# EugenHotaj/zig_gpt2

Hardware: AMD Instinct MI355X
Metric: tokens/sec GPT-2-124M greedy 1024-ctx (higher is better)
Workload: dtype bf16 weights, f32 activations/accumulate; 1 GPU; GPT-2 124M greedy decode, 1 prompt(s)/GPU x 1 GPU(s), 1-token prompts, 1024 decode steps per prompt (reference generate loop, src/main.zig:322-342); vocab=50257, context=1024, n_layer=12, n_heads=12, n_embed=768, prompts_per_gpu=1, global_prompts=1, kv_cache=f32, hip_graph=True, l2_prefetcher=on, parallelism=replicated weights, prompts sharded x1, RCCL broadcast at start-up only

## Files before the change

### zig_gpt2_amd/csrc/elementwise.hip

```cpp
#include <algorithm>

#include "zg_kernels.h"

namespace zg {

namespace {

__device__ __forceinline__ float block_allsum(float v, float* s_red) {
    v = wave_allsum(v);
    const int lane = threadIdx.x & 63, wave = threadIdx.x >> 6, nw = blockDim.x >> 6;
    __syncthreads();
    if (lane == 0) s_red[wave] = v;
    __syncthreads();
    float t = 0.0f;
    for (int w = 0; w < nw; ++w) t += s_red[w];
    return t;
}

__device__ __forceinline__ float block_allmax(float v, float* s_red) {
    v = wave_allmax(v);
    const int lane = threadIdx.x & 63, wave = threadIdx.x >> 6, nw = blockDim.x >> 6;
    __syncthreads();
    if (lane == 0) s_red[wave] = v;
    __syncthreads();
// ... 147 lines not shown
        out[r * n_embed + e] = in[r * 3 * n_embed + split_idx * n_embed + e];
}

__global__ __launch_bounds__(64) void transpose_kernel(const float* in, size_t t, size_t n, size_t h, float* out) {
    const size_t s = blockIdx.x, hh = blockIdx.y, b = blockIdx.z;
    const float* src = in + b * t * n * h + s * n * h + hh * h;
    float* dst = out + b * t * n * h + hh * t * h + s * h;
    for (size_t d = threadIdx.x; d < h; d += blockDim.x) dst[d] = src[d];
}

__global__ __launch_bounds__(256) void copy_kernel(const float* in, float* out, size_t n) {
    const size_t stride = (size_t)gridDim.x * blockDim.x;
    for (size_t i = (size_t)blockIdx.x * blockDim.x + threadIdx.x; i < n; i += stride) out[i] = in[i];
}

__global__ __launch_bounds__(256) void f32_to_bf16_kernel(const float* in, bf16_t* out, size_t n) {
    const size_t stride = (size_t)gridDim.x * blockDim.x;
    for (size_t i = (size_t)blockIdx.x * blockDim.x + threadIdx.x; i < n; i += stride)
        out[i] = f32_to_bf16_rne(in[i]);
}

__global__ __launch_bounds__(256) void split3_kernel(const float* __restrict__ in, bf16_t* __restrict__ out, size_t rows, int K) {
    const size_t quads = rows * (size_t)(K / 4), stride = (size_t)gridDim.x * blockDim.x;
    for (size_t i = (size_t)blockIdx.x * blockDim.x + threadIdx.x; i < quads; i += stride) {
        const size_t r = i / (K / 4), k = (i % (K / 4)) * 4;
        const f32x4 v = *reinterpret_cast<const f32x4*>(in + r * K + k);
        uint32_t h0, m0, l0, h1, m1, l1;
        split3_pk(v.x, v.y, h0, m0, l0);
        split3_pk(v.z, v.w, h1, m1, l1);
        bf16_t* o = out + r * (size_t)(3 * K) + k;
        *reinterpret_cast<u32x2*>(o) = u32x2{h0, h1};
        *reinterpret_cast<u32x2*>(o + K) = u32x2{m0, m1};
        *reinterpret_cast<u32x2*>(o + 2 * K) = u32x2{l0, l1};
    }
}

__device__ __forceinline__ f32x4 load_b24x4(const void* w, size_t row, int K, int k) {
    const char* r = reinterpret_cast<const char*>(w) + row * (size_t)(3 * K);
    const u32x2 h = *reinterpret_cast<const u32x2*>(r + 2 * (size_t)k);
    const uint32_t l = *reinterpret_cast<const uint32_t*>(r + 2 * (size_t)K + k);
    return f32x4{__uint_as_float((h.x << 16) | ((l & 0xffu) << 8)), __uint_as_float((h.x & 0xffff0000u) | (l & 0xff00u)),
                 __uint_as_float((h.y << 16) | ((l >> 8) & 0xff00u)), __uint_as_float((h.y & 0xffff0000u) | ((l >> 16) & 0xff00u))};
}

__global__ __launch_bounds__(256) void f32_to_b24_kernel(const float* __restrict__ in, size_t rows, int K, char* __restrict__ out) {
    const size_t per_row = (size_t)(K / 8), n = rows * per_row;
    for (size_t i = blockIdx.x * (size_t)blockDim.x + threadIdx.x; i < n; i += (size_t)gridDim.x * blockDim.x) {
        const size_t r = i / per_row, k = (i % per_row) * 8;
        const f32x4 a = *reinterpret_cast<const f32x4*>(in + r * K + k);
        const f32x4 b = *reinterpret_cast<const f32x4*>(in + r * K + k + 4);
        const float v[8] = {a.x, a.y, a.z, a.w, b.x, b.y, b.z, b.w};
        uint32_t q[8];
#pragma unroll
        for (int j = 0; j < 8; ++j) q[j] = b24_round(v[j]);
        char* o = out + r * (size_t)(3 * K);
        *reinterpret_cast<u32x4*>(o + 2 * k) = u32x4{(q[0] >> 8) | ((q[1] >> 8) << 16), (q[2] >> 8) | ((q[3] >> 8) << 16),
                                                     (q[4] >> 8) | ((q[5] >> 8) << 16), (q[6] >> 8) | ((q[7] >> 8) << 16)};
        *reinterpret_cast<u32x2*>(o + 2 * (size_t)K + k) =
            u32x2{(q[0] & 0xffu) | (q[1] & 0xffu) << 8 | (q[2] & 0xffu) << 16 | (q[3] & 0xffu) << 24,
                  (q[4] & 0xffu) | (q[5] & 0xffu) << 8 | (q[6] & 0xffu) << 16 | (q[7] & 0xffu) << 24};
    }
}

__global__ __launch_bounds__(256) void b24_split3_kernel(const char* __restrict__ in, size_t rows, int K, bf16_t* __restrict__ out) {
    const size_t per_row = (size_t)(K / 4), n = rows * per_row, total = rows * (size_t)K;
    for (size_t i = blockIdx.x * (size_t)blockDim.x + threadIdx.x; i < n; i += (size_t)gridDim.x * blockDim.x) {
        const size_t r = i / per_row, k = (i % per_row) * 4;
        const f32x4 v = load_b24x4(in, r, K, (int)k);
        uint32_t h0, m0, l0, h1, m1, l1;
        split3_pk(v.x, v.y, h0, m0, l0);
        split3_pk(v.z, v.w, h1, m1, l1);
        bf16_t* o = out + r * K + k;
        *reinterpret_cast<u32x2*>(o) = u32x2{h0, h1};
        *reinterpret_cast<u32x2*>(o + total) = u32x2{m0, m1};
        *reinterpret_cast<u32x2*>(o + 2 * total) = u32x2{l0, l1};
    }
}

__device__ __forceinline__ float load_emb(const void* w, int wt, size_t off) {
    if (wt == WT_BF16) return __uint_as_float((uint32_t)reinterpret_cast<const bf16_t*>(w)[off] << 16);
    return reinterpret_cast<const float*>(w)[off];
}

__global__ __launch_bounds__(512) void embed_step_kernel(const EmbedArgs a) {
    __shared__ int s_tok[8];
    const int lane = threadIdx.x & 63, wave = threadIdx.x >> 6;
    const int s = a.ctrl->step;
    const int mode = a.ctrl->mode;
    const int npart = a.n_partials;
    const int n_waves = a.batch > 4 ? 8 : 4;
    for (int b = wave; b < a.batch; b += n_waves) {
        float bv = -3.0e38f;
        int bi = 0x7fffffff;
        for (int base = 0; base < npart; base += 512) {
            float pv[8];
            int pi[8];
#pragma unroll
            for (int j = 0; j < 8; ++j) {
                const int p = min(base + lane + 64 * j, npart - 1);
                pv[j] = a.part_val[(size_t)b * a.part_stride + p];
                pi[j] = a.part_idx[(size_t)b * a.part_stride + p];
            }
#pragma unroll
            for (int j = 0; j < 8; ++j) {
                if (pv[j] > bv || (pv[j] == bv && pi[j] < bi)) { bv = pv[j]; bi = pi[j]; }
            }
        }
        {
            ZG_PIN(a.forced); ZG_PIN(a.wte); ZG_PIN(a.wpe); ZG_PIN(a.weight_type); ZG_PIN(a.n_embed); ZG_PIN(a.cur_token); ZG_PIN(a.out_tokens);
            ZG_PIN(a.out_stride); ZG_PIN(a.x); ZG_PIN(a.pl_out); ZG_PIN(a.pl_g); ZG_PIN(a.epoch); ZG_PIN(a.finish_only); ZG_PIN(a.st_out); ZG_PIN(a.vocab);
        }
        if (b == 0 && a.progress != nullptr && a.finish_only == 0 && lane == 0) {
            const unsigned xcc = __builtin_amdgcn_s_getreg((3 << 11) | 20) & 7u;
            const unsigned long long word = ((unsigned long long)(0x100u | xcc) << 32) | (((unsigned)(s + 1) << 8) | 1u);
            __hip_atomic_store(static_cast<unsigned long long*>(__builtin_assume_aligned(a.progress, 8)), word, __ATOMIC_RELAXED,
                               __HIP_MEMORY_SCOPE_AGENT);
#ifdef ZG_STAMPS
            reinterpret_cast<PfCtl*>(a.progress)->xcd_log[0] = 0x100u | xcc;
#endif
        }
        const int np = a.prompt_len ? a.prompt_len[b] : 0;
        const int p_cur = a.prompt[(size_t)b * a.prompt_stride + min(s, a.prompt_stride - 1)];
        const int p_last = a.prompt[(size_t)b * a.prompt_stride + max(min(np, a.prompt_stride) - 1, 0)];
        const int forced = a.forced[b];
        const int drawn = a.sampled[b];
#define ZG_AM_STEP(N)                                                                                                   \
    {                                                                                                                   \
        const float ov = dpp_row_ror<N>(bv);                                                                            \
        const int oi = __builtin_amdgcn_update_dpp(0, bi, 0x120 | N, 0xF, 0xF, true);                                   \
        if (ov > bv || (ov == bv && oi < bi)) { bv = ov; bi = oi; }                                                     \
    }
        ZG_AM_STEP(8) ZG_AM_STEP(4) ZG_AM_STEP(2) ZG_AM_STEP(1)
#undef ZG_AM_STEP
        {
            const float rv = bv;
            const int ri = bi;
#pragma unroll
            for (int r = 0; r < 64; r += 16) {
                const float ov = lane_value(rv, r);
                const int oi = __builtin_amdgcn_readlane(ri, r);
                if (ov > bv || (ov == bv && oi < bi)) { bv = ov; bi = oi; }
            }
        }
        int g = (unsigned)bi < (unsigned)a.vocab ? bi : 0;
        if (mode == 2 && a.finish_only != 2) g = (unsigned)drawn < (unsigned)a.vocab ? drawn : 0;
        const bool have_pick = a.finish_only == 2 || ((mode != 1) && (s >= 1) && (s - 1 >= np));
        if (lane == 0) {
            if (have_pick) {
                if (a.finish_only == 2) a.cur_token[b] = g;
                else a.out_tokens[(size_t)b * a.out_stride + (s - 1)] = g;
            }
            if (a.finish_only == 0 || a.finish_only == 3) {
                int tok;
                if (mode == 1) tok = forced;
                else if (s < np) tok = p_cur;
                else if (s == np) tok = p_last;
                else tok = g;
                if (mode != 1 && s < np) a.out_tokens[(size_t)b * a.out_stride + s] = tok;
                a.cur_token[b] = tok;
                s_tok[b] = tok;
            }
        }
    }
    if (a.finish_only == 1 || a.finish_only == 2) return;
    __syncthreads();
    const int total4 = a.batch * (a.n_embed >> 2);
    for (int i = threadIdx.x; i < total4; i += 64 * n_waves) {
        const int b = i / (a.n_embed >> 2), e = (i % (a.n_embed >> 2)) * 4;
        const int tok = s_tok[b];
        f32x4 o;
        if (a.weight_type == WT_BF16) {
            const u32x2 t = *reinterpret_cast<const u32x2*>(reinterpret_cast<const bf16_t*>(a.wte) + (size_t)tok * a.n_embed + e);
            const u32x2 p = *reinterpret_cast<const u32x2*>(reinterpret_cast<const bf16_t*>(a.wpe) + (size_t)s * a.n_embed + e);
            o.x = bf16_lo(t.x) + bf16_lo(p.x);
            o.y = bf16_hi(t.x) + bf16_hi(p.x);
            o.z = bf16_lo(t.y) + bf16_lo(p.y);
            o.w = bf16_hi(t.y) + bf16_hi(p.y);
        } else if (a.weight_type == WT_B24) {
            o = load_b24x4(a.wte, (size_t)tok, a.n_embed, e) + load_b24x4(a.wpe, (size_t)s, a.n_embed, e);
        } else {
            const f32x4 t = *reinterpret_cast<const f32x4*>(reinterpret_cast<const float*>(a.wte) + (size_t)tok * a.n_embed + e);
            const f32x4 p = *reinterpret_cast<const f32x4*>(reinterpret_cast<const float*>(a.wpe) + (size_t)s * a.n_embed + e);
            o = t + p;
        }
        *reinterpret_cast<f32x4*>(a.x + (size_t)b * a.n_embed + e) = o;
        if (a.pl_out) {
            const f32x4 v = o * *reinterpret_cast<const f32x4*>(a.pl_g + e);
            uint32_t h0, m0, l0, h1, m1, l1;
            split3_pk(v.x, v.y, h0, m0, l0);
            split3_pk(v.z, v.w, h1, m1, l1);
            *reinterpret_cast<u32x2*>(a.pl_out + plane_elem(0, b, e)) = u32x2{h0, h1};
            *reinterpret_cast<u32x2*>(a.pl_out + plane_elem(1, b, e)) = u32x2{m0, m1};
            *reinterpret_cast<u32x2*>(a.pl_out + plane_elem(2, b, e)) = u32x2{l0, l1};
        }
        if (a.st_out) {
            float s1 = (o.x + o.y) + (o.z + o.w);
            float s2 = fmaf(o.x, o.x, fmaf(o.y, o.y, fmaf(o.z, o.z, o.w * o.w)));
            s1 += __shfl_xor(s1, 1, 64); s2 += __shfl_xor(s2, 1, 64);
            s1 += __shfl_xor(s1, 2, 64); s2 += __shfl_xor(s2, 2, 64);
            if ((threadIdx.x & 3) == 0) *reinterpret_cast<float2*>(a.st_out + ((size_t)b * (a.n_embed >> 4) + (e >> 4)) * 2) = float2{s1, s2};
        }
    }
    if (threadIdx.x == 0 && a.epoch) *a.epoch += 1u;
    if (threadIdx.x == 0 && a.finish_only == 0) {
        a.ctrl->seq_len = s + 1;
        a.ctrl->step = s + 1;
    }
}

constexpr int kSegMax = 4096;

__global__ __launch_bounds__(256) void sample_seg_kernel(const float* __restrict__ logits, int vocab, const SampleParams* params, float inv_temp_arg,
                                                         const float* __restrict__ part_val, int n_part, int part_stride, float* __restrict__ seg_out) {
    __shared__ float s_red[4];
    const int tid = threadIdx.x, lane = tid & 63, wave = tid >> 6, b = blockIdx.y;
    const float inv_temp = params ? params->inv_temp : inv_temp_arg;
    const float* x = logits + (size_t)b * vocab;
    float* so = seg_out + (size_t)b * (kSegMax + 2);
    float mxr = -3.0e38f;
    for (int p = tid; p < n_part; p += 256) mxr = fmaxf(mxr, part_val[(size_t)b * part_stride + p]);
    mxr = wave_allmax(mxr);
    if (lane == 0) s_red[wave] = mxr;
    __syncthreads();
    const float mx = fmaxf(fmaxf(s_red[0], s_red[1]), fmaxf(s_red[2], s_red[3])) * inv_temp;
    const int nseg = (vocab + 63) >> 6;
    for (int sg = blockIdx.x * 4 + wave; sg < nseg; sg += gridDim.x * 4) {
        const int i = sg * 64 + lane;
        const float e = i < vocab ? __expf(x[i] * inv_temp - mx) : 0.0f;
        const float t = wave_allsum(e);
        if (lane == 0) so[sg] = t;
    }
    if (blockIdx.x == 0 && tid == 0) so[kSegMax] = mx;
}

template <bool FILT>
__global__ __launch_bounds__(64) void sample_pick_kernel(const float* __restrict__ logits, int vocab, const SampleParams* params, float inv_temp_arg,
                                                         const float* __restrict__ u_arr, const StepCtrl* ctrl, float* __restrict__ seg_io,
                                                         int* __restrict__ token_out, const float* __restrict__ tau_arr) {
    const int lane = threadIdx.x, b = blockIdx.x;
    const float tau = FILT ? tau_arr[b] : 0.0f;
    const float inv_temp = params ? params->inv_temp : inv_temp_arg;
    const float* x = logits + (size_t)b * vocab;
    float* so = seg_io + (size_t)b * (kSegMax + 2);
    float u;
    if (u_arr) u = u_arr[b];
    else {
        unsigned long long z = params->seed * 0x9E3779B97F4A7C15ULL + (unsigned long long)ctrl->seq_len * 0xD1B54A32D192ED03ULL + (unsigned long long)b + 1ULL;
        z = (z ^ (z >> 30)) * 0xBF58476D1CE4E5B9ULL;
        z = (z ^ (z >> 27)) * 0x94D049BB133111EBULL;
        z ^= z >> 31;
        u = (float)(unsigned)(z >> 40) * 5.9604644775390625e-08f;
    }
    const int nseg = (vocab + 63) >> 6;
    const int run = (nseg + 63) >> 6, s0 = lane * run, s1 = min(s0 + run, nseg);
    const float mx = so[kSegMax];
    float local = 0.0f;
    for (int k = s0; k < s1; ++k) local += so[k];
    float incl = local;
#pragma unroll
    for (int off = 1; off < 64; off <<= 1) {
        const float up = __shfl_up(incl, off, 64);
        if (lane >= off) incl += up;
    }
    const float total = __shfl(incl, 63, 64);
    const float point = u * total;
    int pick = vocab - 1;
    unsigned long long hit = __builtin_amdgcn_ballot_w64(s0 < s1 && point < incl);
    if (hit != 0ull) {
        const int owner = __builtin_ctzll(hit);
        int sg = 0;
        float before = 0.0f;
        if (lane == owner) {
            before = incl - local;
            sg = s1 - 1;
            for (int k = s0; k < s1; ++k) {
                const float v = so[k];
                if (point < before + v) {
                    sg = k;
                    break;
                }
                before += v;
            }
        }
        sg = __shfl(sg, owner, 64);
        before = __shfl(before, owner, 64);
        const int i = sg * 64 + lane;
        const float xi = i < vocab ? x[i] : 0.0f;
        const bool kept = i < vocab && (!FILT || xi >= tau);
        float c = kept ? __expf(FILT ? (xi - mx) * inv_temp : xi * inv_temp - mx) : 0.0f;
// ... 299 lines not shown
                                       2 * kPenMaxHistory * 2 * (int)sizeof(unsigned)));
            raised = true;
        }
    }
    hipLaunchKernelGGL(penalty_apply_kernel, dim3(batch), dim3(256), lds, s, logits, vocab, params, h, slots, counts_out);
    ZG_HIP(hipGetLastError());
    hipLaunchKernelGGL(row_argmax_partials_kernel, dim3(n_part, batch), dim3(256), 0, s, logits, vocab, part_val, part_idx);
    ZG_HIP(hipGetLastError());
    return ZG_OK;
}

static inline int logprob_chunks(int vocab) { return (vocab + kLpChunk - 1) / kLpChunk; }

size_t logprob_workspace_bytes(int batch, int vocab) { return (size_t)batch * logprob_chunks(vocab) * (1 + 2 * kLpTopMax) * 4; }

LogprobWs logprob_workspace(void* base, int batch, int vocab) {
    const size_t slots = (size_t)batch * logprob_chunks(vocab);
    LogprobWs w;
    w.sum = static_cast<float*>(base);
    w.val = w.sum + slots;
    w.idx = reinterpret_cast<int*>(w.val + slots * kLpTopMax);
    return w;
}

int launch_logprob(const float* logits, int batch, int vocab, const float* part_val, const int* part_idx, int n_part, int part_stride, const int* top_n,
                   const LogprobWs& ws, const int* tokens, const StepCtrl* ctrl, const int* prompt_len, const LogprobRec& rec, hipStream_t s) {
    ZG_REQUIRE(vocab >= 1 && vocab <= kLpChunk * kLpMaxChunks, ZG_ERR_UNSUPPORTED, "log-probabilities: vocabulary of %d beyond %d", vocab,
               kLpChunk * kLpMaxChunks);
    ZG_REQUIRE(logits && part_val && (tokens || part_idx) && n_part >= 1 && top_n && ws.sum && rec.logprob && rec.top_ids && rec.top_logprobs &&
                   rec.stride >= 1 && batch >= 1,
               ZG_ERR_ARG, "log-probabilities: missing argument");
    const int nc = logprob_chunks(vocab);
    hipLaunchKernelGGL(logprob_part_kernel, dim3(nc, batch), dim3(256), 0, s, logits, vocab, part_val, n_part, part_stride, top_n, ws, nc);
    ZG_HIP(hipGetLastError());
    hipLaunchKernelGGL(logprob_finish_kernel, dim3(batch), dim3(256), 0, s, logits, vocab, part_val, part_idx, n_part, part_stride, top_n, ws, nc, tokens,
                       ctrl, prompt_len, rec);
    ZG_HIP(hipGetLastError());
    return ZG_OK;
}

size_t score_workspace_bytes(int rows, int vocab) { return (size_t)rows * logprob_chunks(vocab) * (2 + 2 * kLpTopMax) * 4; }

ScoreWs score_workspace(void* base, int rows, int vocab) {
    const size_t slots = (size_t)rows * logprob_chunks(vocab);
    ScoreWs w;
    w.lp.sum = static_cast<float*>(base);
    w.max = w.lp.sum + slots;
    w.lp.val = w.max + slots;
    w.lp.idx = reinterpret_cast<int*>(w.lp.val + slots * kLpTopMax);
    return w;
}

int launch_score(const float* logits, int rows, int vocab, int row_stride, const int* top_n, const ScoreWs& ws, const ScoreTargets& tg, const LogprobRec& rec,
                 hipStream_t s) {
    ZG_REQUIRE(vocab >= 1 && vocab <= kLpChunk * kLpMaxChunks, ZG_ERR_UNSUPPORTED, "score: vocabulary of %d beyond %d", vocab, kLpChunk * kLpMaxChunks);
    ZG_REQUIRE(logits && top_n && ws.lp.sum && tg.tokens && tg.token_stride >= 1 && tg.n >= 1 && tg.past >= 0 && tg.row0 >= 0 && rec.logprob && rec.top_ids &&
                   rec.top_logprobs && rec.stride >= 1 && rows >= 1 && rows <= 65535 && row_stride >= vocab,
               ZG_ERR_ARG, "score: missing argument");
    const int nc = logprob_chunks(vocab);
    hipLaunchKernelGGL(score_part_kernel, dim3(nc, rows), dim3(256), 0, s, logits, vocab, row_stride, top_n, ws, nc);
    ZG_HIP(hipGetLastError());
    hipLaunchKernelGGL(score_finish_kernel, dim3(rows), dim3(256), 0, s, logits, vocab, row_stride, top_n, ws, nc, tg, rec);
    ZG_HIP(hipGetLastError());
    return ZG_OK;
}

int launch_stop(const StopArgs& a, hipStream_t s) {
    ZG_REQUIRE(a.conds && a.tokens && a.prompt_len && a.finish_col && a.reason && a.stride >= 1 && a.batch >= 1 && a.batch <= kStopMaxRows && a.vocab >= 1 &&
                   (a.col >= 0 ? a.col < a.stride : a.ctrl != nullptr) && (a.picks || a.pick_from_record || (a.part_val && a.part_idx && a.n_part >= 1)),
               ZG_ERR_ARG, "stop stage: missing argument");
    hipLaunchKernelGGL(stop_step_kernel, dim3(1), dim3(a.batch > 4 ? 512 : 256), 0, s, a);
    ZG_HIP(hipGetLastError());
    return ZG_OK;
}

int launch_wte_planes(const void* wte, int weight_type, size_t V, size_t V64, int K, bf16_t* out, hipStream_t s) {
    ZG_REQUIRE(wte && out && V >= 1 && V64 >= V && K % 8 == 0 && (weight_type == WT_F32 || weight_type == WT_B24), ZG_ERR_ARG, "wte planes: bad argument");
    hipLaunchKernelGGL(wte_planes_kernel, dim3(grid_for(V64 * (size_t)(K / 4))), dim3(256), 0, s, wte, weight_type, V, V64, K, out);
    ZG_HIP(hipGetLastError());
    return ZG_OK;
}

int launch_embed_step(const EmbedArgs& a, hipStream_t s) {
    hipLaunchKernelGGL(embed_step_kernel, dim3(1), dim3(a.batch > 4 ? 512 : 256), 0, s, a);
    ZG_HIP(hipGetLastError());
    return ZG_OK;
}

}
```

### zig_gpt2_amd/csrc/gemv.hip

```cpp
#include "gemv_internal.h"

namespace zg {

namespace {

struct Rung {
    int max, lpr, cpl;
};
constexpr Rung kValuLadder[] = {{32, 16, 2}, {64, 16, 4}, {96, 16, 6}, {128, 16, 8}, {192, 32, 6}, {256, 32, 8}, {384, 64, 6}, {512, 64, 8}, {1024, 64, 16}};
constexpr Rung kKsplitLadder[] = {{32, 16, 2}, {96, 32, 3}, {160, 32, 5}, {224, 32, 7}, {256, 64, 4}};
constexpr Rung kLnkLadder[] = {{32, 16, 2}, {64, 32, 2}, {96, 32, 3}, {128, 64, 2}};
template <int N>
inline Rung rung(const Rung (&ladder)[N], int chunks) {
    for (const Rung& r : ladder)
        if (chunks <= r.max) return r;
    return Rung{0, 64, 0};
}

inline int ceil_div(int a, int b) { return (a + b - 1) / b; }

inline int valu_mt(int M) { return M <= 1 ? 1 : (M <= 2 ? 2 : (M <= 4 ? 4 : 8)); }
inline size_t valu_lds(int strips, int mt, int K) { return ((size_t)strips * K + 4 * mt * 2 + 64) * sizeof(float); }

void plan_valu(const GemvArgs& a, GemvPlan& p) {
// ... 17 lines not shown
    p.lds = (int)valu_lds(mt == 1 ? wpw : mt, mt, a.K);
    p.rows_per_wg = a.M > 1 ? 0 : wpw * p.rows_per_wave;
    p.pf_tiles = a.M > 1 ? 0 : p.grid;
    p.supported = p.mt != 0 && p.cpl != 0 && (size_t)p.lds <= kGemvLdsMax;
    if (a.K % 8 != 0) {
        p = GemvPlan{};
        p.route = GR_GENERIC, p.grid = ceil_div(a.N, 4), p.kslices = 1, p.block = 256, p.waves_per_wg = 4;
        p.supported = a.prologue == PRO_NONE && a.epilogue == EPI_STORE;
    }
}

inline size_t mfma_lds(int K, int nw, bool alias, bool line, bool gpl) {
    const size_t planes = gpl ? 0 : (size_t)3 * kMfmaRows * (2 * K + 16);
    return planes + 64 * sizeof(float) + (alias ? 0 : (size_t)2 * nw * 64 * 4 * sizeof(float)) + (line ? (size_t)nw * 2048 : 0);
}

bool plan_mfma(const GemvArgs& a, int off, GemvPlan& p) {
    const bool argmax = a.epilogue == EPI_ARGMAX, ln = a.prologue == PRO_LAYERNORM;
    const int ntiles = ceil_div(a.N, 16);
    const bool sliced = a.sk_ws != nullptr && a.sk_cnt != nullptr && a.prologue == PRO_NONE && !argmax && a.epilogue != EPI_QKV &&
                        a.K >= 2048 && a.K % 128 == 0 && a.K / 4 <= 3072 && ntiles <= a.sk_tiles;
    if (!sliced) {
        if (a.K % 32 != 0 || a.K / 32 < 4 || a.K / 32 > 96 || (ln && a.K > 2048)) return false;
        const bool wide_ok = !argmax && ntiles <= 768 && mfma_lds(a.K, 16, true, false, false) <= kGemvLdsMax;
        if (mfma_lds(a.K, argmax ? 4 : 16, false, false, false) > kGemvLdsMax && !wide_ok) return false;
    }
    p.supported = true;
    p.can_write_planes = !argmax;
    p.can_take_planes = !argmax && (a.prologue == PRO_NONE || (ln && a.ln_c2 != nullptr && a.ln_c3 != nullptr && a.K <= 2048));
    p.kslices = sliced ? 4 : 1;
    const int Ks = a.K / p.kslices, steps = Ks / 32;
    const bool wpt = !(off & 32) && argmax && ln && (steps == 12 || steps == 24 || steps == 32);
    p.rows_per_wave = sliced ? 1 : (wpt ? 8 : ceil_div(ntiles, 768));
    if (p.rows_per_wave < 1) p.rows_per_wave = 1;
    p.grid = ceil_div(ntiles, p.rows_per_wave);
    p.rows_per_wg = sliced ? 0 : 16 * p.rows_per_wave;
    p.pf_tiles = sliced ? 0 : p.grid;
    const int pairs = (Ks / 64 + 3) / 4;
    const bool pl4_shape = !(off & 2) && !argmax && p.rows_per_wave == 1 && a.N <= 0xffff && !(ln && a.x_stride != a.K) &&
                           !(a.epilogue == EPI_RESIDUAL && a.resid_stride != a.N) && !(a.st_in != nullptr && a.K / 16 > 128) &&
                           a.K % (64 * p.kslices) == 0 && pairs >= 1 && pairs <= 5;
    p.pl4_with_planes = p.can_take_planes && pl4_shape;
    p.waves_per_wg = 4;
    p.block = 256;
    const bool planes = a.pl_in != nullptr && p.can_take_planes;
    if (planes && pl4_shape) {
        p.route = sliced ? GR_PL4_KS : GR_PL4;
        p.pairs = pairs;
    } else if (wpt) {
        p.route = GR_LM_WPT;
        p.steps = steps;
        p.lds = (int)((size_t)3 * kMfmaRows * (2 * a.K + 16) + 4 * kMfmaRows * 8 + 4 * 4096);
    } else {
        p.route = sliced ? GR_MFMA16_KS : GR_MFMA16;
        p.nw = argmax ? 4 : 16;
        const int per_wave = ceil_div(steps, p.nw);
        if (argmax) p.ks = per_wave <= 3 ? 3 : (per_wave <= 6 ? 6 : (per_wave <= 13 ? 13 : 24));
        else p.ks = per_wave <= 2 ? 2 : (per_wave <= 4 ? 4 : 6);
        p.gpl = planes;
        p.alias = !p.gpl && !sliced && !argmax && p.rows_per_wave == 1 && mfma_lds(a.K, 16, false, false, false) > kGemvLdsMax;
        p.line = !(off & 16) && !p.alias && Ks % 64 == 0 && mfma_lds(Ks, p.nw, false, true, p.gpl) <= kGemvLdsMax;
        p.lds = (int)mfma_lds(Ks, p.nw, p.alias, p.line, p.gpl);
        p.waves_per_wg = p.nw;
        p.block = 64 * p.nw;
    }
    return true;
}

}

GemvPlan gemv_plan(const GemvArgs& a, int weight_type) {
    GemvPlan p{};
    const int off = decode_paths_off();
    if (weight_type == WT_BF16 && a.M >= 2 && a.M <= kMfmaRows && plan_mfma(a, off, p)) return p;
    plan_valu(a, p);
    const bool plain_epi = a.epilogue == EPI_STORE || a.epilogue == EPI_RESIDUAL || a.epilogue == EPI_GELU;
    const int nchq = a.K / 32;
    auto take = [&p](int route, const Rung& r, int passes) { p.route = route, p.lpr = r.lpr, p.cpl = r.cpl, p.rows_per_wg = passes * (64 / r.lpr); };
    if (a.M == 1 && plain_epi && a.K % 32 == 0 &&
        (a.prologue == PRO_ATTN_MERGE
             ? a.head_dim == 64 && a.t_hi > 0 && ceil_div(a.t_hi, kAttnChunk) <= 4 && a.K <= 1024
             : a.prologue == PRO_NONE && a.K >= 2048 && nchq <= 256)) {
        take(GR_KSPLIT, rung(kKsplitLadder, nchq), 2);
    } else if (a.M == 1 && a.prologue == PRO_LAYERNORM && a.ln_c2 != nullptr && a.ln_c3 != nullptr &&
               (a.epilogue == EPI_STORE || a.epilogue == EPI_GELU || a.epilogue == EPI_QKV) && a.K % 32 == 0 && nchq <= 128 && a.N <= 16384) {
        take(GR_LNK, rung(kLnkLadder, nchq), 4);
    } else if (a.M > 1 && valu_lds(valu_mt(a.M), valu_mt(a.M), a.K) > kGemvLdsMax && a.prologue == PRO_NONE && plain_epi) {
        int g = valu_mt(a.M);
        while (g > 1 && valu_lds(g, g, a.K) > kGemvLdsMax) g >>= 1;
        GemvArgs b = a;
        b.M = g;
        plan_valu(b, p);
        p.route = GR_VALU_GROUPS, p.row_group = g;
        p.rows_per_wg = p.pf_tiles = 0;
    }
    if (p.route != GR_KSPLIT && p.route != GR_LNK) return p.supported ? p : GemvPlan{};
    p.rows_per_wave = p.rows_per_wg, p.waves_per_wg = 4;
    p.grid = ceil_div(a.N, p.rows_per_wg), p.block = 256, p.lds = 0;
    p.supported = true;
    return p;
}

int launch_gemv(const GemvArgs& a, const GemvPlan& p, int weight_type, hipStream_t s) {
    ZG_REQUIRE(a.pl_in == nullptr || p.can_take_planes, ZG_ERR_UNSUPPORTED, "gemv: input planes given to a launch outside the matrix-core path");
    ZG_REQUIRE(a.pl_out == nullptr || p.can_write_planes, ZG_ERR_UNSUPPORTED, "gemv: output planes asked of a launch outside the matrix-core path");
    ZG_REQUIRE(p.supported, ZG_ERR_UNSUPPORTED,
               "gemv: no kernel for M=%d x K=%d, prologue %d, epilogue %d (at most 8 rows per launch that fit the LDS, whole or in groups; K <= 8192; "
               "K not a multiple of 8 only for a plain Linear)", a.M, a.K, a.prologue, a.epilogue);
    GemvArgs b = a;
    b.rows_per_wave = p.rows_per_wave;
    b.waves_per_wg = p.alias ? -1 : p.waves_per_wg;
    b.kslices = p.kslices;
    switch (p.route) {
        case GR_KSPLIT: return gemv_launch_ksplit(b, p, weight_type, s);
        case GR_LNK: return gemv_launch_lnk(b, p, weight_type, s);
        case GR_MFMA16: case GR_MFMA16_KS: return gemv_launch_mfma16(b, p, s);
        case GR_PL4: case GR_PL4_KS: return gemv_launch_pl4(b, p, s);
        case GR_LM_WPT: return gemv_launch_lm_wpt(b, p, s);
        case GR_VALU_GROUPS:
            for (int m0 = 0; m0 < a.M; m0 += p.row_group) {
                b.M = a.M - m0 < p.row_group ? a.M - m0 : p.row_group;
                b.x = a.x + (size_t)m0 * a.x_stride;
                b.y = a.y + (size_t)m0 * a.y_stride;
                if (a.resid) b.resid = a.resid + (size_t)m0 * a.resid_stride;
                GemvPlan q{};
                plan_valu(b, q);
                b.rows_per_wave = q.rows_per_wave, b.waves_per_wg = q.waves_per_wg;
                ZG_TRY(gemv_launch_valu(b, q, weight_type, s));
            }
            return ZG_OK;
        default: return gemv_launch_valu(b, p, weight_type, s);
    }
}

}
```

### zig_gpt2_amd/csrc/gemv_ksplit.hip

```cpp
#include "gemv_internal.h"

namespace zg {

namespace {

template <typename WT, int LPR, int CPL, int NP = 2>
__global__ __launch_bounds__(256) void gemv_ksplit_kernel(const void* __restrict__ Wv, const float* __restrict__ xin, int N,
                                                          int K, unsigned em, const float* __restrict__ part_in, int max_splits,
                                                          const float* __restrict__ bias, const float* __restrict__ resid,
                                                          const GemvArgs a) {
    const int epilogue = (int)(em & 0xffu), merge_splits = (int)((em >> 8) & 0xffu);
    const int has_bias = (int)((em >> 16) & 1u), has_resid = (int)((em >> 17) & 1u);
    ZG_STAMP_DECL();
    ZG_STAMP(0);
    constexpr int RPP = 64 / LPR, ROWS = NP * RPP;
    __shared__ float part[4][ROWS];
    const int tid = threadIdx.x, lane = tid & 63;
    const int wave = __builtin_amdgcn_readfirstlane(tid >> 6);
    const int lr = lane % LPR, rsub = lane / LPR;
    const int Kq = K >> 2, nchq = Kq >> 3;
    const auto W = wmat<WT>(Wv, (size_t)wave * Kq);
    const int row0 = blockIdx.x * ROWS;
    Raw<WT> wq[NP][CPL];
#pragma unroll
    for (int p = 0; p < NP; ++p) {
        const auto pr = wrow(W, (size_t)min(row0 + p * RPP + rsub, N - 1), K);
#pragma unroll
        for (int i = 0; i < CPL; ++i) wq[p][i] = load_raw(pr, min(lr + LPR * i, nchq - 1));
    }
    W8 xr[CPL];
    if (merge_splits > 0) {
        constexpr int MAXS = 4;
        const int nsplit = merge_splits;
#pragma unroll
        for (int i = 0; i < CPL; ++i) {
            const int e0 = wave * Kq + min(lr + LPR * i, nchq - 1) * 8;
            const int h = e0 >> 6, d0 = e0 & 63;
            const float* p = part_in + ((size_t)h * max_splits) * kPartStride;
            float ms[MAXS], ls[MAXS];
            W8 o[MAXS];
#pragma unroll
            for (int sp = 0; sp < MAXS; ++sp) {
                const float* ps = p + min(sp, nsplit - 1) * kPartStride;
                ms[sp] = ps[64];
                ls[sp] = ps[65];
                const float2 a0 = *reinterpret_cast<const float2*>(ps + d0), a1 = *reinterpret_cast<const float2*>(ps + d0 + 2);
                const float2 a2 = *reinterpret_cast<const float2*>(ps + d0 + 4), a3 = *reinterpret_cast<const float2*>(ps + d0 + 6);
                o[sp].v[0] = a0.x; o[sp].v[1] = a0.y; o[sp].v[2] = a1.x; o[sp].v[3] = a1.y;
                o[sp].v[4] = a2.x; o[sp].v[5] = a2.y; o[sp].v[6] = a3.x; o[sp].v[7] = a3.y;
            }
#pragma unroll
            for (int sp = 0; sp < MAXS; ++sp)
                if (sp >= nsplit) ms[sp] = -1e30f;
            const float mx = fmaxf(fmaxf(ms[0], ms[1]), fmaxf(ms[2], ms[3]));
            float l = 0.0f;
            W8 r = zero_w8();
#pragma unroll
            for (int sp = 0; sp < MAXS; ++sp) {
                const float w = __expf(ms[sp] - mx);
                l = fmaf(w, ls[sp], l);
#pragma unroll
                for (int j = 0; j < 8; ++j) r.v[j] = fmaf(w, o[sp].v[j], r.v[j]);
            }
            const float inv = 1.0f / l;
#pragma unroll
            for (int j = 0; j < 8; ++j) xr[i].v[j] = r.v[j] * inv;
        }
    } else {
#pragma unroll
        for (int i = 0; i < CPL; ++i) xr[i] = load_x8(xin + (size_t)wave * Kq + (size_t)min(lr + LPR * i, nchq - 1) * 8);
    }
    float bias_n = 0.0f, resid_n = 0.0f;
    if (tid < ROWS) {
        const int n = min(row0 + tid, N - 1);
        bias_n = bias[n * has_bias];
        resid_n = resid[n * has_resid];
    }
    ZG_STAMP(1);
    ZG_PIN(a.y);
    ZG_PIN(a.progress);
    pf_count(a.progress);
    ZG_STAMP(2);
#pragma unroll
    for (int i = 0; i < CPL; ++i)
        if (lr + LPR * i >= nchq) xr[i] = zero_w8();
    auto dot = [&](const Raw<WT>(&w)[CPL]) {
        float p0 = 0.0f, p1 = 0.0f, p2 = 0.0f, p3 = 0.0f;
#pragma unroll
        for (int i = 0; i < CPL; ++i) {
            const W8 u = unpack(w[i]);
            p0 = fmaf(u.v[0], xr[i].v[0], p0); p1 = fmaf(u.v[1], xr[i].v[1], p1);
            p2 = fmaf(u.v[2], xr[i].v[2], p2); p3 = fmaf(u.v[3], xr[i].v[3], p3);
            p0 = fmaf(u.v[4], xr[i].v[4], p0); p1 = fmaf(u.v[5], xr[i].v[5], p1);
            p2 = fmaf(u.v[6], xr[i].v[6], p2); p3 = fmaf(u.v[7], xr[i].v[7], p3);
        }
        return group_allsum<LPR>((p0 + p1) + (p2 + p3));
    };
    float sp[NP];
#pragma unroll
    for (int p = 0; p < NP; ++p) sp[p] = dot(wq[p]);
    ZG_STAMP(3);
    if (lr == 0) {
#pragma unroll
        for (int p = 0; p < NP; ++p) part[wave][p * RPP + rsub] = sp[p];
    }
    __syncthreads();
    ZG_STAMP(4);
    if (tid < ROWS && row0 + tid < N) {
        const int n = row0 + tid;
        const float v = ((part[0][tid] + part[1][tid]) + (part[2][tid] + part[3][tid])) + bias_n;
        a.y[n] = epilogue == EPI_RESIDUAL ? v + resid_n : (epilogue == EPI_GELU ? gelu_ref(v) : v);
    }
    ZG_STAMP(5);
    ZG_STAMP(6);
    ZG_STAMP(7);
    ZG_STAMP_FLUSH();
}

template <typename WT>
int launch_ksplit(const GemvArgs& a, const GemvPlan& pl, hipStream_t s) {
    const int merge_splits = a.prologue == PRO_ATTN_MERGE ? (a.t_hi + kAttnChunk - 1) / kAttnChunk : 0;
    const unsigned has_resid = a.epilogue == EPI_RESIDUAL ? 1u : 0u;
    const unsigned em = (unsigned)a.epilogue | ((unsigned)merge_splits << 8) | ((a.bias ? 1u : 0u) << 16) | (has_resid << 17);
#define ZG_KS(LPR_, CPL_)                                                                                                \
    if (pl.lpr == LPR_ && pl.cpl == CPL_) {                                                                              \
        note_kernel("gemv_ksplit_kernel<%s, %d, %d, 2>", wt_name<WT>(), LPR_, CPL_);         \
        hipLaunchKernelGGL((gemv_ksplit_kernel<WT, LPR_, CPL_, 2>), dim3(pl.grid), dim3(256), 0, s, a.W,                     \
                           a.x,                                                                                         \
                           a.N, a.K, em, a.part ? a.part : a.zero, a.max_splits, a.bias ? a.bias : a.zero,              \
                           has_resid ? a.resid : a.zero, a);                                                             \
        ZG_HIP(hipGetLastError());                                                                                       \
        return ZG_OK;                                                                                                    \
    }
    ZG_KS(16, 2)
    ZG_KS(32, 3)
    ZG_KS(32, 5)
    ZG_KS(32, 7)
    ZG_KS(64, 4)
#undef ZG_KS
    zg::set_error("gemv (K split): no instantiation for K=%d", a.K);
    return ZG_ERR_UNSUPPORTED;
}


template <typename WT, int LPR, int CPL, int NP = 2>
__global__ __launch_bounds__(256) void gemv_lnk_kernel(const void* __restrict__ Wv, const float* __restrict__ xin, unsigned ne, int K,
                                                       const float* __restrict__ ln_g, const float* __restrict__ c2,
                                                       const float* __restrict__ c3, const int* __restrict__ cw,
                                                       const GemvArgs a) {
    gemv_lnk_body<WT, LPR, CPL, NP, false>((int)blockIdx.x, Wv, xin, ne, K, ln_g, c2, c3, cw, a, 1u, nullptr, nullptr, 0u);
}

template <typename WT>
__global__ __launch_bounds__(256) void ln_fold_kernel(const void* __restrict__ Wv, const float* __restrict__ g,
                                                      const float* __restrict__ b, const float* __restrict__ bias, int N, int K,
                                                      float* __restrict__ c2, float* __restrict__ c3) {
    const int lane = threadIdx.x & 63, row = blockIdx.x * 4 + (threadIdx.x >> 6);
    if (row >= N) return;
    const WT* w = reinterpret_cast<const WT*>(Wv) + (size_t)row * K;
    float s2 = 0.0f, s3 = 0.0f;
    for (int k = lane; k < K; k += 64) {
        float wv;
        if constexpr (sizeof(WT) == 2) wv = __uint_as_float((uint32_t)w[k] << 16);
        else if constexpr (sizeof(WT) == 3) wv = b24_elem(Wv, (size_t)row, K, (size_t)k);
        else wv = w[k];
        s2 = fmaf(wv, g[k], s2);
        s3 = fmaf(wv, b[k], s3);
    }
    s2 = wave_allsum(s2);
    s3 = wave_allsum(s3);
    if (lane == 0) {
        c2[row] = s2;
        c3[row] = s3 + (bias ? bias[row] : 0.0f);
    }
}

template <typename WT>
int launch_lnk(const GemvArgs& a, const GemvPlan& pl, hipStream_t s) {
#define ZG_LK(LPR_, CPL_)                                                                                              \
    if (pl.lpr == LPR_ && pl.cpl == CPL_) {                                                                            \
        note_kernel("gemv_lnk_kernel<%s, %d, %d, 4>", wt_name<WT>(), LPR_, CPL_);       \
        hipLaunchKernelGGL((gemv_lnk_kernel<WT, LPR_, CPL_, 4>), dim3(pl.grid), dim3(256), 0, s, a.W, a.x,             \
                           (unsigned)a.N | ((unsigned)a.epilogue << 24), a.K, a.ln_g, a.ln_c2, a.ln_c3,                 \
                           a.ctrl ? reinterpret_cast<const int*>(a.ctrl) : reinterpret_cast<const int*>(a.zero), a);   \
        ZG_HIP(hipGetLastError());                                                                                     \
        return ZG_OK;                                                                                                  \
    }
    ZG_LK(16, 2)
    ZG_LK(32, 2)
    ZG_LK(32, 3)
    ZG_LK(64, 2)
#undef ZG_LK
    zg::set_error("gemv (LayerNorm, K split): no instantiation for K=%d", a.K);
    return ZG_ERR_UNSUPPORTED;
}



}

int gemv_launch_ksplit(const GemvArgs& a, const GemvPlan& p, int weight_type, hipStream_t s) {
    if (weight_type == WT_B24) return launch_ksplit<b24_t>(a, p, s);
    return weight_type == WT_BF16 ? launch_ksplit<bf16_t>(a, p, s) : launch_ksplit<float>(a, p, s);
}
int gemv_launch_lnk(const GemvArgs& a, const GemvPlan& p, int weight_type, hipStream_t s) {
    if (weight_type == WT_B24) return launch_lnk<b24_t>(a, p, s);
    return weight_type == WT_BF16 ? launch_lnk<bf16_t>(a, p, s) : launch_lnk<float>(a, p, s);
}

int launch_ln_fold(const void* W, int weight_type, const float* g, const float* b, const float* bias, int N, int K, float* c2,
                   float* c3, hipStream_t s) {
    if (weight_type == WT_BF16)
        hipLaunchKernelGGL((ln_fold_kernel<bf16_t>), dim3((N + 3) / 4), dim3(256), 0, s, W, g, b, bias, N, K, c2, c3);
    else if (weight_type == WT_B24)
        hipLaunchKernelGGL((ln_fold_kernel<b24_t>), dim3((N + 3) / 4), dim3(256), 0, s, W, g, b, bias, N, K, c2, c3);
    else
        hipLaunchKernelGGL((ln_fold_kernel<float>), dim3((N + 3) / 4), dim3(256), 0, s, W, g, b, bias, N, K, c2, c3);
    ZG_HIP(hipGetLastError());
    return ZG_OK;
}

}
```

### zig_gpt2_amd/csrc/zg_kernels.h

```cpp
#pragma once
#include "zg_common.h"

namespace zg {

struct StepCtrl {
    int step;
    int seq_len;
    int mode;
    int n_partials;
};

enum GemvPrologue { PRO_NONE = 0, PRO_LAYERNORM = 1, PRO_ATTN_MERGE = 2 };
enum GemvEpilogue { EPI_STORE = 0, EPI_RESIDUAL = 1, EPI_GELU = 2, EPI_QKV = 3, EPI_ARGMAX = 4 };
enum WeightType { WT_BF16 = 0, WT_F32 = 1, WT_B24 = 2  };

constexpr int kAttnChunk = 256;
constexpr int kPartStride = 64 + 2;

struct GemvArgs {
    const void* W;
    const float* bias;
    int N, K, M;
    int rows_per_wave;
    int waves_per_wg;
    int prologue, epilogue;
    const float* x;
    int x_stride;
    const float* ln_g;
    const float* ln_b;
    float eps;
    const float* ln_c2;
    const float* ln_c3;
    const float* part;
    int n_heads, head_dim, max_splits;
    const StepCtrl* ctrl;
    int t_hi;
    float* y;
    int y_stride;
    const float* resid;
    int resid_stride;
    float* q;
    void* k_cache;
    void* v_cache;
    int ctx;
    int kv_mode;
    size_t kv_lo;
    float* logits;
    int logits_stride;
    float* part_val;
    int* part_idx;
    float* sk_ws;
    int* sk_cnt;
    int sk_tiles;
    int kslices;
    const bf16_t* pl_in;
    bf16_t* pl_out;
    const float* pl_g;
    const unsigned* epoch;
    unsigned launch_id;
    unsigned long long* sk_tag;
    unsigned* fault;
    unsigned spin_limit;
    float* st_out;
    const float* st_in;
    const float* zero;
    unsigned long long* dbg;
    unsigned* progress;
};

enum GemvRoute {
    GR_VALU = 0,
    GR_VALU_GROUPS = 1,
    GR_GENERIC = 2,
    GR_KSPLIT = 3,
    GR_LNK = 4,
    GR_MFMA16 = 5,
    GR_MFMA16_KS = 6,
    GR_PL4 = 7,
    GR_PL4_KS = 8,
    GR_LM_WPT = 9,
};
struct GemvPlan {
    int route;
    int grid, kslices;
    int block;
    int lds;
    int mt, lpr, cpl;
    int ks, nw;
    bool line, gpl, alias;
    int pairs;
    int steps;
    int rows_per_wave;
    int waves_per_wg;
    int row_group;
    int rows_per_wg, pf_tiles;
    bool supported;
    bool can_take_planes;
    bool can_write_planes;
    bool pl4_with_planes;
};
GemvPlan gemv_plan(const GemvArgs& a, int weight_type);
int launch_gemv(const GemvArgs& a, const GemvPlan& p, int weight_type, hipStream_t s);
int launch_ln_fold(const void* W, int weight_type, const float* g, const float* b, const float* bias, int N, int K, float* c2,
                   float* c3, hipStream_t s);

struct AttnArgs {
    const float* q;
    const void* k;
    const void* v;
    long stride_b, stride_h, stride_t;
    int kv_mode;
    size_t kv_lo;
    int n_heads, head_dim, batch;
    const StepCtrl* ctrl;
    int seq_len;
    int t_hi;
    int max_splits;
    float* part;
    unsigned* progress;
    bf16_t* pl_out;
    int* merge_cnt;
    const unsigned* epoch;
    unsigned launch_id;
    unsigned long long* part_tag;
    unsigned* fault;
    unsigned spin_limit;
};
int launch_attn_decode(const AttnArgs& a, hipStream_t s);
bool attn_qkv_ok(const GemvArgs& g, const GemvPlan& p, const AttnArgs& at);
int launch_attn_qkv(const GemvArgs& g, const GemvPlan& p, int weight_type, const AttnArgs& at, const unsigned* epoch, unsigned long long* qkv_tag, hipStream_t s);
int launch_attn_any_dim(const float* q, const float* k, const float* v, long stride_b, long stride_h, long stride_t, int batch, int n_heads,
                        int head_dim, int seq_len, float* out, hipStream_t s);
int launch_attn_merge(const float* part, int batch, int n_heads, int head_dim, int max_splits,
                      int seq_len, float* out, hipStream_t s);

int launch_epoch_bump(unsigned* epoch, hipStream_t s);
int launch_layernorm(float* x, int rows, int n, const float* g, const float* b, float eps, hipStream_t s, unsigned* done_flag = nullptr,
                     unsigned done_seq = 0, bool* announced = nullptr, float* shadow = nullptr);
int launch_gelu(float* x, size_t n, hipStream_t s, unsigned* done_flag = nullptr, unsigned done_seq = 0, bool* announced = nullptr, float* shadow = nullptr);
int launch_softmax(float* x, size_t n, hipStream_t s, unsigned* done_flag = nullptr, unsigned done_seq = 0, bool* announced = nullptr);
int launch_done_flag(unsigned* flag, unsigned seq, hipStream_t s);
struct CopySegs {
    const void* src[4];
    void* dst[4];
    unsigned bytes[4];
    int n;
};
int launch_copy_out_done(const CopySegs& segs, unsigned* flag, unsigned seq, hipStream_t s);
int launch_copy2_f32(const float* a, float* da, const float* b, float* db, size_t n, hipStream_t s);
int launch_embedding(const float* w, size_t emb_dim, const size_t* idx, size_t n_idx, size_t n_rows,
                     float* out, int* d_oob_flag, hipStream_t s, unsigned* done_flag = nullptr, unsigned done_seq = 0, bool* announced = nullptr);
int launch_split_qkv(const float* in, size_t rows, size_t n_embed, size_t split_idx, float* out, hipStream_t s);
int launch_transpose(const float* in, size_t batch, size_t t, size_t n, size_t h, float* out, hipStream_t s);
int launch_copy_f32(const float* in, float* out, size_t n, hipStream_t s);
int launch_f32_to_bf16(const float* in, bf16_t* out, size_t n, hipStream_t s);
int launch_split3(const float* in, size_t rows, int K, bf16_t* out, hipStream_t s);
int launch_f32_to_b24(const float* in, size_t rows, int K, void* out, hipStream_t s);
int launch_b24_split3(const void* in, size_t rows, int K, bf16_t* out, hipStream_t s);
int launch_kv_clear_tail(void* base, int n_caches, size_t cache_stride, size_t plane_off, int row_bytes, int strips, int ctx, int from_row,
                         hipStream_t s);

int launch_gemm_bf16_nt(const bf16_t* A, const bf16_t* B, const float* bias, void* C, int M, int N, int K, int ldc,
                        bool gelu, bool out_bf16, hipStream_t s);
struct GemmPlanes {
    int lda, ldb;
    int kpp;
    int npairs;
    unsigned pa_bits, pb_bits;
    bool b_plane_major;
};
int launch_gemm_planes(const bf16_t* A, const bf16_t* B, const float* bias, void* C, int M, int N, const GemmPlanes& pl,
                       int ldc, bool gelu, bool out_bf16, hipStream_t s);
int launch_gemm_s4(const bf16_t* A, const bf16_t* B, const float* bias, void* C, int M, int N, const GemmPlanes& pl, int ldc,
                   bool gelu, bool out_bf16, int bn, hipStream_t s);
bool gemm_s4_args_ok(const GemmPlanes& pl, int ldc);
struct S4Grid {
    int grid, band, lds;
};
int gemm_s4_wg_cap();
S4Grid gemm_s4_grid(int items, int tiles_n, int wg_cap);
enum { S4_PLAIN = 0, S4_PARTIAL = 1, S4_QKV = 2, S4_SPLIT3 = 3 };
struct PrefillQkv;
// ... 270 lines not shown
```

Baseline: 5052 tokens/s.

## Specialize attention-merge ksplit GEMV on split count and hoist per-head softmax stats

Templates the k-split GEMV attention-merge prologue on the number of attention splits (1-4) so the merge loop is fully unrolled with no clamped padding splits. Per-head max/sum statistics are preloaded once per wave into registers instead of being reloaded for every chunk. The generic path stays as a fallback selectable by plan bits. Separately, the embed/argmax step kernel now receives its hot fields as scalar kernel arguments rather than from the args struct, which changes where it reads them from. The cost is more kernel instantiations and some extra register pressure.

```diff
diff --git a/zig_gpt2_amd/csrc/elementwise.hip b/zig_gpt2_amd/csrc/elementwise.hip
--- a/zig_gpt2_amd/csrc/elementwise.hip
+++ b/zig_gpt2_amd/csrc/elementwise.hip
@@ -253,14 +253,15 @@
     return reinterpret_cast<const float*>(w)[off];
 }
 
-__global__ __launch_bounds__(512) void embed_step_kernel(const EmbedArgs a) {
+__global__ __launch_bounds__(512) void embed_step_kernel(StepCtrl* ctrl, const float* part_val, const int* part_idx, int part_stride, int n_partials,
+                                                         const int* prompt, const int* prompt_len, int batch, int prompt_stride, const EmbedArgs a) {
     __shared__ int s_tok[8];
     const int lane = threadIdx.x & 63, wave = threadIdx.x >> 6;
-    const int s = a.ctrl->step;
-    const int mode = a.ctrl->mode;
-    const int npart = a.n_partials;
-    const int n_waves = a.batch > 4 ? 8 : 4;
-    for (int b = wave; b < a.batch; b += n_waves) {
+    const int s = ctrl->step;
+    const int mode = ctrl->mode;
+    const int npart = n_partials;
+    const int n_waves = batch > 4 ? 8 : 4;
+    for (int b = wave; b < batch; b += n_waves) {
         float bv = -3.0e38f;
         int bi = 0x7fffffff;
         for (int base = 0; base < npart; base += 512) {
@@ -269,17 +270,18 @@
 #pragma unroll
             for (int j = 0; j < 8; ++j) {
                 const int p = min(base + lane + 64 * j, npart - 1);
-                pv[j] = a.part_val[(size_t)b * a.part_stride + p];
-                pi[j] = a.part_idx[(size_t)b * a.part_stride + p];
+                pv[j] = part_val[(size_t)b * part_stride + p];
+                pi[j] = part_idx[(size_t)b * part_stride + p];
+            }
+            {
+                ZG_PIN(a.forced); ZG_PIN(a.wte); ZG_PIN(a.wpe); ZG_PIN(a.weight_type); ZG_PIN(a.n_embed); ZG_PIN(a.cur_token); ZG_PIN(a.out_tokens);
+                ZG_PIN(a.out_stride); ZG_PIN(a.x); ZG_PIN(a.pl_out); ZG_PIN(a.pl_g); ZG_PIN(a.epoch); ZG_PIN(a.finish_only); ZG_PIN(a.st_out); ZG_PIN(a.vocab);
+                ZG_PIN(a.progress); ZG_PIN(a.sampled);
             }
 #pragma unroll
             for (int j = 0; j < 8; ++j) {
                 if (pv[j] > bv || (pv[j] == bv && pi[j] < bi)) { bv = pv[j]; bi = pi[j]; }
             }
-        }
-        {
-            ZG_PIN(a.forced); ZG_PIN(a.wte); ZG_PIN(a.wpe); ZG_PIN(a.weight_type); ZG_PIN(a.n_embed); ZG_PIN(a.cur_token); ZG_PIN(a.out_tokens);
-            ZG_PIN(a.out_stride); ZG_PIN(a.x); ZG_PIN(a.pl_out); ZG_PIN(a.pl_g); ZG_PIN(a.epoch); ZG_PIN(a.finish_only); ZG_PIN(a.st_out); ZG_PIN(a.vocab);
         }
         if (b == 0 && a.progress != nullptr && a.finish_only == 0 && lane == 0) {
             const unsigned xcc = __builtin_amdgcn_s_getreg((3 << 11) | 20) & 7u;
@@ -290,9 +292,9 @@
             reinterpret_cast<PfCtl*>(a.progress)->xcd_log[0] = 0x100u | xcc;
 #endif
         }
-        const int np = a.prompt_len ? a.prompt_len[b] : 0;
-        const int p_cur = a.prompt[(size_t)b * a.prompt_stride + min(s, a.prompt_stride - 1)];
-        const int p_last = a.prompt[(size_t)b * a.prompt_stride + max(min(np, a.prompt_stride) - 1, 0)];
+        const int np = prompt_len ? prompt_len[b] : 0;
+        const int p_cur = prompt[(size_t)b * prompt_stride + min(s, prompt_stride - 1)];
+        const int p_last = prompt[(size_t)b * prompt_stride + max(min(np, prompt_stride) - 1, 0)];
         const int forced = a.forced[b];
         const int drawn = a.sampled[b];
 #define ZG_AM_STEP(N)                                                                                                   \
@@ -335,7 +337,7 @@
     }
     if (a.finish_only == 1 || a.finish_only == 2) return;
     __syncthreads();
-    const int total4 = a.batch * (a.n_embed >> 2);
+    const int total4 = batch * (a.n_embed >> 2);
     for (int i = threadIdx.x; i < total4; i += 64 * n_waves) {
         const int b = i / (a.n_embed >> 2), e = (i % (a.n_embed >> 2)) * 4;
         const int tok = s_tok[b];
@@ -374,8 +376,8 @@
     }
     if (threadIdx.x == 0 && a.epoch) *a.epoch += 1u;
     if (threadIdx.x == 0 && a.finish_only == 0) {
-        a.ctrl->seq_len = s + 1;
-        a.ctrl->step = s + 1;
+        ctrl->seq_len = s + 1;
+        ctrl->step = s + 1;
     }
 }
 
@@ -841,9 +843,10 @@
 }
 
 int launch_embed_step(const EmbedArgs& a, hipStream_t s) {
-    hipLaunchKernelGGL(embed_step_kernel, dim3(1), dim3(a.batch > 4 ? 512 : 256), 0, s, a);
-    ZG_HIP(hipGetLastError());
-    return ZG_OK;
-}
-
-}
+    hipLaunchKernelGGL(embed_step_kernel, dim3(1), dim3(a.batch > 4 ? 512 : 256), 0, s, a.ctrl, a.part_val, a.part_idx, a.part_stride, a.n_partials,
+                       a.prompt, a.prompt_len, a.batch, a.prompt_stride, a);
+    ZG_HIP(hipGetLastError());
+    return ZG_OK;
+}
+
+}
diff --git a/zig_gpt2_amd/csrc/gemv.hip b/zig_gpt2_amd/csrc/gemv.hip
--- a/zig_gpt2_amd/csrc/gemv.hip
+++ b/zig_gpt2_amd/csrc/gemv.hip
@@ -123,6 +123,7 @@
              ? a.head_dim == 64 && a.t_hi > 0 && ceil_div(a.t_hi, kAttnChunk) <= 4 && a.K <= 1024
              : a.prologue == PRO_NONE && a.K >= 2048 && nchq <= 256)) {
         take(GR_KSPLIT, rung(kKsplitLadder, nchq), 2);
+        p.merge_generic = (off & 128) != 0, p.merge_ml_vector = (off & 256) != 0;
     } else if (a.M == 1 && a.prologue == PRO_LAYERNORM && a.ln_c2 != nullptr && a.ln_c3 != nullptr &&
                (a.epilogue == EPI_STORE || a.epilogue == EPI_GELU || a.epilogue == EPI_QKV) && a.K % 32 == 0 && nchq <= 128 && a.N <= 16384) {
         take(GR_LNK, rung(kLnkLadder, nchq), 4);
diff --git a/zig_gpt2_amd/csrc/gemv_ksplit.hip b/zig_gpt2_amd/csrc/gemv_ksplit.hip
--- a/zig_gpt2_amd/csrc/gemv_ksplit.hip
+++ b/zig_gpt2_amd/csrc/gemv_ksplit.hip
@@ -1,10 +1,23 @@
+#include <algorithm>
+
 #include "gemv_internal.h"
 
 namespace zg {
 
 namespace {
 
-template <typename WT, int LPR, int CPL, int NP = 2>
+constexpr int kNsGeneric = 5;
+
+__device__ __forceinline__ W8 load_part8(const float* ps, int d0) {
+    const float2 a0 = *reinterpret_cast<const float2*>(ps + d0), a1 = *reinterpret_cast<const float2*>(ps + d0 + 2);
+    const float2 a2 = *reinterpret_cast<const float2*>(ps + d0 + 4), a3 = *reinterpret_cast<const float2*>(ps + d0 + 6);
+    W8 o;
+    o.v[0] = a0.x; o.v[1] = a0.y; o.v[2] = a1.x; o.v[3] = a1.y;
+    o.v[4] = a2.x; o.v[5] = a2.y; o.v[6] = a3.x; o.v[7] = a3.y;
+    return o;
+}
+
+template <typename WT, int LPR, int CPL, int NP, int NS, int NH>
 __global__ __launch_bounds__(256) void gemv_ksplit_kernel(const void* __restrict__ Wv, const float* __restrict__ xin, int N,
                                                           int K, unsigned em, const float* __restrict__ part_in, int max_splits,
                                                           const float* __restrict__ bias, const float* __restrict__ resid,
@@ -13,6 +26,7 @@
     const int has_bias = (int)((em >> 16) & 1u), has_resid = (int)((em >> 17) & 1u);
     ZG_STAMP_DECL();
     ZG_STAMP(0);
+    static_assert(NS >= 0 && NS <= kNsGeneric && NH >= 0 && NH <= 4 && (NH == 0 || (NS >= 1 && NS <= 4)), "see the table above");
     constexpr int RPP = 64 / LPR, ROWS = NP * RPP;
     __shared__ float part[4][ROWS];
     const int tid = threadIdx.x, lane = tid & 63;
@@ -29,7 +43,60 @@
         for (int i = 0; i < CPL; ++i) wq[p][i] = load_raw(pr, min(lr + LPR * i, nchq - 1));
     }
     W8 xr[CPL];
-    if (merge_splits > 0) {
+    if constexpr (NS >= 1 && NS < kNsGeneric) {
+        float2 mlh[NH > 0 ? NH : 1][NS];
+        const int h0w = (wave * Kq) >> 6;
+        if constexpr (NH > 0) {
+            const int hlast = (K >> 6) - 1;
+#pragma unroll
+            for (int j = 0; j < NH; ++j) {
+                const int hj = min(h0w + j, hlast);
+#pragma unroll
+                for (int sp = 0; sp < NS; ++sp)
+                    mlh[j][sp] = *reinterpret_cast<const float2*>(part_in + ((size_t)hj * max_splits + sp) * kPartStride + 64);
+            }
+        }
+#pragma unroll
+        for (int i = 0; i < CPL; ++i) {
+            const int e0 = wave * Kq + min(lr + LPR * i, nchq - 1) * 8;
+            const int h = e0 >> 6, d0 = e0 & 63;
+            const float* p = part_in + ((size_t)h * max_splits) * kPartStride;
+            float ms[NS], ls[NS];
+            W8 o[NS];
+#pragma unroll
+            for (int sp = 0; sp < NS; ++sp) {
+                const float* ps = p + sp * kPartStride;
+                o[sp] = load_part8(ps, d0);
+                if constexpr (NH == 0) {
+                    ms[sp] = ps[64];
+                    ls[sp] = ps[65];
+                } else {
+                    float2 ml = mlh[0][sp];
+#pragma unroll
+                    for (int j = 1; j < NH; ++j)
+                        if (h - h0w >= j) ml = mlh[j][sp];
+                    ms[sp] = ml.x;
+                    ls[sp] = ml.y;
+                }
+            }
+            float mx = ms[0];
+            if constexpr (NS == 2) mx = fmaxf(ms[0], ms[1]);
+            if constexpr (NS == 3) mx = fmaxf(fmaxf(ms[0], ms[1]), ms[2]);
+            if constexpr (NS == 4) mx = fmaxf(fmaxf(ms[0], ms[1]), fmaxf(ms[2], ms[3]));
+            float l = 0.0f;
+            W8 r = zero_w8();
+#pragma unroll
+            for (int sp = 0; sp < NS; ++sp) {
+                const float w = __expf(ms[sp] - mx);
+                l = fmaf(w, ls[sp], l);
+#pragma unroll
+                for (int j = 0; j < 8; ++j) r.v[j] = fmaf(w, o[sp].v[j], r.v[j]);
+            }
+            const float inv = 1.0f / l;
+#pragma unroll
+            for (int j = 0; j < 8; ++j) xr[i].v[j] = r.v[j] * inv;
+        }
+    } else if constexpr (NS == kNsGeneric) {
         constexpr int MAXS = 4;
         const int nsplit = merge_splits;
 #pragma unroll
@@ -44,10 +111,7 @@
                 const float* ps = p + min(sp, nsplit - 1) * kPartStride;
                 ms[sp] = ps[64];
                 ls[sp] = ps[65];
-                const float2 a0 = *reinterpret_cast<const float2*>(ps + d0), a1 = *reinterpret_cast<const float2*>(ps + d0 + 2);
-                const float2 a2 = *reinterpret_cast<const float2*>(ps + d0 + 4), a3 = *reinterpret_cast<const float2*>(ps + d0 + 6);
-                o[sp].v[0] = a0.x; o[sp].v[1] = a0.y; o[sp].v[2] = a1.x; o[sp].v[3] = a1.y;
-                o[sp].v[4] = a2.x; o[sp].v[5] = a2.y; o[sp].v[6] = a3.x; o[sp].v[7] = a3.y;
+                o[sp] = load_part8(ps, d0);
             }
 #pragma unroll
             for (int sp = 0; sp < MAXS; ++sp)
@@ -122,23 +186,35 @@
     const int merge_splits = a.prologue == PRO_ATTN_MERGE ? (a.t_hi + kAttnChunk - 1) / kAttnChunk : 0;
     const unsigned has_resid = a.epilogue == EPI_RESIDUAL ? 1u : 0u;
     const unsigned em = (unsigned)a.epilogue | ((unsigned)merge_splits << 8) | ((a.bias ? 1u : 0u) << 16) | (has_resid << 17);
-#define ZG_KS(LPR_, CPL_)                                                                                                \
-    if (pl.lpr == LPR_ && pl.cpl == CPL_) {                                                                              \
-        note_kernel("gemv_ksplit_kernel<%s, %d, %d, 2>", wt_name<WT>(), LPR_, CPL_);         \
-        hipLaunchKernelGGL((gemv_ksplit_kernel<WT, LPR_, CPL_, 2>), dim3(pl.grid), dim3(256), 0, s, a.W,                     \
-                           a.x,                                                                                         \
+    int ns = merge_splits, nh = 0;
+    if (merge_splits > 0 && (pl.merge_generic || merge_splits > 4)) ns = kNsGeneric;
+    if (ns >= 1 && ns <= 4 && !pl.merge_ml_vector) {
+        const int Kq = a.K >> 2;
+        for (int w = 0; w < 4; ++w) nh = std::max(nh, (((w + 1) * Kq - 1) >> 6) - ((w * Kq) >> 6) + 1);
+        if (nh > Kq / 64 + 1 || nh > 4) nh = 0;
+    }
+#define ZG_KS(LPR_, CPL_, NS_, NH_)                                                                                      \
+    if (pl.lpr == LPR_ && pl.cpl == CPL_ && ns == NS_ && nh == NH_) {                                                    \
+        note_kernel("gemv_ksplit_kernel<%s, %d, %d, 2, %d, %d>", wt_name<WT>(), LPR_, CPL_, NS_, NH_);                   \
+        hipLaunchKernelGGL((gemv_ksplit_kernel<WT, LPR_, CPL_, 2, NS_, NH_>), dim3(pl.grid), dim3(256), 0, s, a.W, a.x,  \
                            a.N, a.K, em, a.part ? a.part : a.zero, a.max_splits, a.bias ? a.bias : a.zero,              \
                            has_resid ? a.resid : a.zero, a);                                                             \
         ZG_HIP(hipGetLastError());                                                                                       \
         return ZG_OK;                                                                                                    \
     }
-    ZG_KS(16, 2)
-    ZG_KS(32, 3)
-    ZG_KS(32, 5)
-    ZG_KS(32, 7)
-    ZG_KS(64, 4)
+#define ZG_KS_MERGE(NS_) ZG_KS(16, 2, NS_, 0) ZG_KS(16, 2, NS_, 1) ZG_KS(16, 2, NS_, 2) ZG_KS(16, 2, NS_, 3) ZG_KS(16, 2, NS_, 4)
+    ZG_KS_MERGE(1)
+    ZG_KS_MERGE(2)
+    ZG_KS_MERGE(3)
+    ZG_KS_MERGE(4)
+    ZG_KS(16, 2, kNsGeneric, 0)
+    ZG_KS(32, 3, 0, 0)
+    ZG_KS(32, 5, 0, 0)
+    ZG_KS(32, 7, 0, 0)
+    ZG_KS(64, 4, 0, 0)
+#undef ZG_KS_MERGE
 #undef ZG_KS
-    zg::set_error("gemv (K split): no instantiation for K=%d", a.K);
+    zg::set_error("gemv (K split): no instantiation for K=%d, %d merge splits", a.K, merge_splits);
     return ZG_ERR_UNSUPPORTED;
 }
 
diff --git a/zig_gpt2_amd/csrc/zg_kernels.h b/zig_gpt2_amd/csrc/zg_kernels.h
--- a/zig_gpt2_amd/csrc/zg_kernels.h
+++ b/zig_gpt2_amd/csrc/zg_kernels.h
@@ -98,6 +98,7 @@
     bool can_take_planes;
     bool can_write_planes;
     bool pl4_with_planes;
+    bool merge_generic, merge_ml_vector;
 };
 GemvPlan gemv_plan(const GemvArgs& a, int weight_type);
 int launch_gemv(const GemvArgs& a, const GemvPlan& p, int weight_type, hipStream_t s);
```

New measurement: 5256 tokens/s (median of 6 runs). 1.04x the previous value.
